# berkeley-hipie/HIPIE

Measured on AMD Instinct MI355X. Metric: images/sec @1024x1024 ViT-H bs=8 (single-image inference hot path: box, class and mask logits), higher is better.
Workload: dtype f16x3 (split-fp16 operands, fp32 accumulate: fp32-class); 1 GPU; BASELINE.json configs[2]: vit_huge, 1024x1024, batch 8 per GPU, 80 class prompts (L=194), detection; global_batch=8, parallelism=dp1, precision_policy=split, launch=eager

## Files before the change

### hipie_amd/csrc/vit_attn_split.hip

```cpp
#include <stdlib.h>

#include "common.h"
#include "mfma.h"
#include "wave.h"

#ifndef HIPIE_VS_TAIL
#define HIPIE_VS_TAIL 1
#endif
#ifndef HIPIE_VS_TAIL_MAXNB
#define HIPIE_VS_TAIL_MAXNB 3
#endif

namespace hipie {

constexpr float VS_LAZY = 6.f;

struct VSParams {
  const f16_t* qkv; f16_t* out; const f16_t* tab_h; const f16_t* tab_w;
  int B, H, N, kh, kw;
  long sb, st;
  long o_sb, o_st;
  int nqt, swz;
  int tr, kwm;
  long krs, kts;
};

template <int HD, int NB, int WAVES, int R, int KW, int BHC>
__global__ __launch_bounds__(WAVES * 64, (NB >= 3 ? 1 : 2)) void vit_attn_split_kernel(const VSParams p) {
  typedef f16_t T;
  constexpr int KT = 32 * NB;
  constexpr int KS = HD / 16;
  constexpr int DB = (HD + 31) / 32;
  constexpr int KSTR = HD + 8;
  constexpr int VSTR = (DB * 32 == 96 || DB * 32 == 32) ? DB * 32 : DB * 32 + 32;
  constexpr int CPR = HD / 8;
  constexpr int KCH = KSTR / 8, VCH = VSTR / 8;
  constexpr int KBLK = (KT * KCH + 63) / 64, VBLK = (KT * VCH + 63) / 64;
  constexpr int KPL = KBLK * 512, VPL = VBLK * 512;
  constexpr int BUF = 2 * KPL + 2 * VPL;
  constexpr int NBLK = 2 * KBLK + 2 * VBLK;
  constexpr int NDMA = (NBLK + WAVES - 1) / WAVES;
  constexpr int QW = WAVES * 32;
  constexpr int NT = WAVES * 64;
  constexpr bool TAIL = (HD % 32 == 16) && (HIPIE_VS_TAIL != 0) && NB <= HIPIE_VS_TAIL_MAXNB;
  constexpr int DBB = TAIL ? HD / 32 : DB;
  constexpr bool ONES = (DB * 32 > HD) && !TAIL;
  static_assert(R == 1 || (KW > 0 && R * KW <= KT), "R key rows of KW keys must fit the tile");
  static_assert(BHC == 0 || (R == 1 && BHC <= 31), "chunked bias_h: one key row per tile, at most 31 rows per chunk");
  static_assert(KSTR % 8 == 0 && VSTR % 8 == 0, "plane rows are whole 16-byte chunks");
  typedef Mfma32<T>::frag frag;
  typedef Mfma32<T>::half_frag hfrag;

  extern __shared__ __attribute__((aligned(1024))) char smem_raw[];
  T* smem = reinterpret_cast<T*>(smem_raw);
  constexpr size_t TILE_BYTES = ((size_t)2 * BUF * sizeof(T) > (size_t)WAVES * 4096) ? (size_t)2 * BUF * sizeof(T) : (size_t)WAVES * 4096;
  float* bh_all = reinterpret_cast<float*>(smem_raw + TILE_BYTES);

  const int tid = threadIdx.x, lane = tid & 63;
  const int wave = __builtin_amdgcn_readfirstlane(tid >> 6);
  const int li = lane & 31, hi = lane >> 5;
  const int kw = (R > 1) ? KW : p.kw, kh = p.kh;

  int bh, qt;
  {
    const int id = blockIdx.x;
    if (p.swz) { bh = (id & 7) + 8 * ((id >> 3) / p.nqt); qt = (id >> 3) % p.nqt; }
    else { bh = id / p.nqt; qt = id % p.nqt; }
  }
  const int b = bh / p.H, h = bh % p.H;
  const long C2 = 2L * p.H * HD;
  const T* Qg = p.qkv + b * p.sb + (long)h * (2 * HD);
  const T* Kg = Qg + C2;
  T* Og = p.out + b * p.o_sb + (long)h * (2 * HD);

  const int qi = qt * QW + wave * 32 + li;
  const int qc = min(qi, p.N - 1);
  const int qy = qc / kw, qx = qc - qy * kw;
  const long qm = p.tr ? (long)qx * p.kwm + qy : (long)qc;
  const int nkt = R * kw;

  frag qh[KS], ql[KS];
#pragma unroll
  for (int ks = 0; ks < KS; ++ks) {
    const T* s = Qg + qm * p.st + 16 * (2 * ks + hi);
    qh[ks] = *reinterpret_cast<const frag*>(s);
    ql[ks] = *reinterpret_cast<const frag*>(s + 8);
  }

  f32x16 bw[NB];
#pragma unroll
  for (int blk = 0; blk < NB; ++blk)
#pragma unroll
    for (int r = 0; r < 16; ++r) bw[blk][r] = -INFINITY;
  {
    float* stage = reinterpret_cast<float*>(smem_raw) + wave * (32 * 32);
    const int nbw = (2 * kw - 1 + 31) / 32, nbh = (2 * kh - 1 + 31) / 32;
    auto table_block = [&](const T* tab, const int rows, const int jb) -> f32x16 {
      f32x16 acc;
#pragma unroll
      for (int r = 0; r < 16; ++r) acc[r] = 0.f;
      const T* ap = tab + (long)min(32 * jb + li, rows - 1) * (2 * HD) + 16 * hi;
#pragma unroll
      for (int ks = 0; ks < KS; ++ks) {
        const frag th = *reinterpret_cast<const frag*>(ap + 32 * ks), tl = *reinterpret_cast<const frag*>(ap + 32 * ks + 8);
        acc = Mfma32<T>::mma(tl, qh[ks], acc);
        acc = Mfma32<T>::mma(th, ql[ks], acc);
        acc = Mfma32<T>::mma(th, qh[ks], acc);
      }
      return acc;
    };
    for (int jb = 0; jb < nbw; ++jb) {
      const f32x16 acc = table_block(p.tab_w, 2 * kw - 1, jb);
#pragma unroll
      for (int r = 0; r < 16; ++r) stage[crow(r, hi) * 32 + li] = acc[r];
      __syncthreads();
#pragma unroll
      for (int blk = 0; blk < NB; ++blk)
#pragma unroll
        for (int r = 0; r < 16; ++r) {
          const int slot = 32 * blk + crow(r, hi);
          const int kx = (R > 1) ? slot % kw : slot;
          const int j = qx + kw - 1 - kx - 32 * jb;
          if (slot < R * kw && j >= 0 && j < 32) bw[blk][r] = stage[j * 32 + li];
        }
      __syncthreads();
    }
    if (BHC == 0) {
      for (int jb = 0; jb < nbh; ++jb) {
        const f32x16 acc = table_block(p.tab_h, 2 * kh - 1, jb);
#pragma unroll
        for (int r = 0; r < 16; ++r) {
          const int ky = qy + kh - 1 - (32 * jb + crow(r, hi));
          if (ky >= 0 && ky < kh) bh_all[ky * QW + wave * 32 + li] = acc[r];
        }
      }
    }
    __syncthreads();
  }
  const int qy0 = __builtin_amdgcn_readfirstlane(qy);
  auto bias_h_chunk = [&](const int t0) {
    const int j0 = qy0 + kh - 1 - (t0 + BHC - 1);
    f32x16 acc;
#pragma unroll
    for (int r = 0; r < 16; ++r) acc[r] = 0.f;
    const T* ap = p.tab_h + (long)min(max(j0 + li, 0), 2 * kh - 2) * (2 * HD) + 16 * hi;
#pragma unroll
    for (int ks = 0; ks < KS; ++ks) {
      const frag th = *reinterpret_cast<const frag*>(ap + 32 * ks), tl = *reinterpret_cast<const frag*>(ap + 32 * ks + 8);
      acc = Mfma32<T>::mma(tl, qh[ks], acc);
      acc = Mfma32<T>::mma(th, ql[ks], acc);
      acc = Mfma32<T>::mma(th, qh[ks], acc);
    }
#pragma unroll
    for (int r = 0; r < 16; ++r) {
      const int ky = qy + kh - 1 - (j0 + crow(r, hi));
      if (ky >= t0 && ky < t0 + BHC && ky < kh) bh_all[(ky - t0) * QW + wave * 32 + li] = acc[r];
    }
  };

  const int nt = (kh + R - 1) / R;
  const bool ragged = (R > 1) && (nt * nkt > p.N);
  auto dma_voff = [&](const int r, const int maxrow) -> unsigned int {
    const int j = wave + WAVES * r;
    const int jj = min(j, NBLK - 1);
    const bool isk = jj < 2 * KBLK;
    const int pl = isk ? jj / KBLK : (jj - 2 * KBLK) / VBLK;
    const int c = 64 * (isk ? jj - pl * KBLK : jj - 2 * KBLK - pl * VBLK) + lane;
    const int nch = isk ? KCH : VCH;
    const int row = min(min(c / nch, KT - 1), maxrow);
    int col = c % nch;
    if (col >= CPR) col = 0;
    return (unsigned int)(((long)row * p.krs + (isk ? 0 : C2) + 16 * col + 8 * pl) * (long)sizeof(T));
  };
  unsigned int dvoff[NDMA];
  unsigned long long dmask[NDMA];
#pragma unroll
  for (int r = 0; r < NDMA; ++r) {
    dvoff[r] = dma_voff(r, nkt - 1);
    const int jj = min(wave + WAVES * r, NBLK - 1);
    const bool isk = jj < 2 * KBLK;
    const int pl = isk ? jj / KBLK : (jj - 2 * KBLK) / VBLK;
    const int c = 64 * (isk ? jj - pl * KBLK : jj - 2 * KBLK - pl * VBLK) + lane;
    dmask[r] = __builtin_amdgcn_ballot_w64(c % (isk ? KCH : VCH) < CPR);
  }
  const unsigned int lds0 = (unsigned int)reinterpret_cast<uintptr_t>((__attribute__((address_space(3))) char*)smem_raw);
  const char* kbase0 = reinterpret_cast<const char*>(Kg);
  const long tile_bytes = (R > 1 ? (long)nkt * p.st : p.kts) * (long)sizeof(T);
  auto dma_tile = [&](const int t, const int buf, const int r) {
    const int j = (WAVES * r + WAVES - 1 < NBLK) ? wave + WAVES * r : min(wave + WAVES * r, NBLK - 1);
    const bool last_ragged = ragged && (t == nt - 1);
    const unsigned int vo = last_ragged ? dma_voff(r, p.N - t * nkt - 1) : dvoff[r];
    const unsigned int ldst = __builtin_amdgcn_readfirstlane(lds0 + (unsigned int)(buf * BUF * (int)sizeof(T) + 1024 * j));
    dma16_masked(kbase0 + (long)t * tile_bytes, vo, ldst, dmask[r]);
  };

  {
    constexpr int PADC = VCH - CPR;
    for (int idx = tid; idx < 2 * 2 * KT * PADC; idx += NT) {
      const int pc = idx % PADC, row = (idx / PADC) % KT, pl = (idx / (PADC * KT)) & 1, buf = idx / (2 * PADC * KT);
      f16x8 z;
#pragma unroll
      for (int e = 0; e < 8; ++e) z[e] = (T)0.f;
      if (ONES && pl == 0 && pc == 0) z[0] = (T)1.f;
      *reinterpret_cast<f16x8*>(smem + buf * BUF + 2 * KPL + pl * VPL + row * VSTR + (CPR + pc) * 8) = z;
    }
  }

  f32x16 O[DBB];
  f32x4 OT[2];
  float m_run = -INFINITY, l_run = 0.f;
#pragma unroll
  for (int d = 0; d < DBB; ++d)
#pragma unroll
    for (int r = 0; r < 16; ++r) O[d][r] = 0.f;
#pragma unroll
  for (int r = 0; r < 4; ++r) { OT[0][r] = 0.f; OT[1][r] = 0.f; }

#pragma unroll
  for (int r = 0; r < NDMA; ++r) dma_tile(0, 0, r);
  __builtin_amdgcn_s_waitcnt(vmcnt(0));
  __syncthreads();

  const int l16 = lane & 15, g1 = (lane >> 4) & 1;
  const int vlane = (4 * hi + (l16 >> 2)) * VSTR + 16 * g1 + 4 * (l16 & 3);
  const int klane = li * KSTR + 8 * hi;

  for (int t = 0; t < nt; ++t) {
    const T* Kh = smem + (t & 1) * BUF;
    const T* Kl = Kh + KPL;
    const T* Vh = Kh + 2 * KPL;
    const T* Vl = Vh + VPL;
    const int tn = min(t + 1, nt - 1);
    if (BHC > 0 && t % (BHC > 0 ? BHC : 1) == 0) bias_h_chunk(t);
    float bh0 = bh_all[(BHC > 0 ? t % (BHC > 0 ? BHC : 1) : R * t) * QW + wave * 32 + li], bh1 = 0.f;
    if (R > 1) bh1 = (R * t + 1 < kh) ? bh_all[(R * t + 1) * QW + wave * 32 + li] : -INFINITY;

    f32x16 S[NB];
    {
      frag kfh[2][NB], kfl[2][NB];
#pragma unroll
      for (int blk = 0; blk < NB; ++blk) {
        kfh[0][blk] = *reinterpret_cast<const frag*>(Kh + klane + 32 * blk * KSTR);
        kfl[0][blk] = *reinterpret_cast<const frag*>(Kl + klane + 32 * blk * KSTR);
      }
#pragma unroll
      for (int ks = 0; ks < KS; ++ks) {
        if (ks + 1 < KS) {
#pragma unroll
          for (int blk = 0; blk < NB; ++blk) {
            kfh[(ks + 1) & 1][blk] = *reinterpret_cast<const frag*>(Kh + klane + 32 * blk * KSTR + 16 * (ks + 1));
            kfl[(ks + 1) & 1][blk] = *reinterpret_cast<const frag*>(Kl + klane + 32 * blk * KSTR + 16 * (ks + 1));
          }
        }
#pragma unroll
        for (int blk = 0; blk < NB; ++blk) {
          S[blk] = Mfma32<T>::mma(kfl[ks & 1][blk], qh[ks], (ks == 0) ? bw[blk] : S[blk]);
          S[blk] = Mfma32<T>::mma(kfh[ks & 1][blk], ql[ks], S[blk]);
          S[blk] = Mfma32<T>::mma(kfh[ks & 1][blk], qh[ks], S[blk]);
        }
        if (ks < NDMA) dma_tile(tn, (t + 1) & 1, ks);
      }
#pragma unroll
      for (int r = KS; r < NDMA; ++r) dma_tile(tn, (t + 1) & 1, r);
    }
    hfrag va[2][DBB], vb[2][DBB];
#pragma unroll
    for (int d = 0; d < DBB; ++d) {
      va[0][d] = Mfma32<T>::tr_read(Vh + vlane + 32 * d);
      vb[0][d] = Mfma32<T>::tr_read(Vh + vlane + 32 * d + 8 * VSTR);
    }

    if (R > 1) {
#pragma unroll
      for (int blk = 0; blk < NB; ++blk)
#pragma unroll
        for (int r = 0; r < 16; ++r) S[blk][r] += (32 * blk + crow(r, hi) < kw) ? bh0 : bh1;
    }
    float t0 = __builtin_fmaxf(S[0][0], S[0][1]);
#pragma unroll
    for (int blk = 1; blk < NB; ++blk) t0 = __builtin_fmaxf(t0, S[blk][0]);
    float mx = t0, mxb = t0, mxc = t0, mxd = t0;
#pragma unroll
    for (int blk = 0; blk < NB; ++blk)
#pragma unroll
      for (int r = 0; r < 16; r += 8) {
        mx = max3(mx, S[blk][r], S[blk][r + 1]);
        mxb = max3(mxb, S[blk][r + 2], S[blk][r + 3]);
        mxc = max3(mxc, S[blk][r + 4], S[blk][r + 5]);
        mxd = max3(mxd, S[blk][r + 6], S[blk][r + 7]);
      }
    mx = max3(mx, mxb, mxc);
    mx = max3(mx, mxd, mxd);
    mx = xhalf_max(mx);
    mx += (R > 1 ? 0.f : bh0);
    if (__builtin_amdgcn_ballot_w64(mx > m_run + VS_LAZY) != 0ull) {
      const float m_new = fmaxf(m_run, mx);
      const float alpha = __builtin_amdgcn_exp2f(m_run - m_new);
      m_run = m_new;
      if (!ONES) l_run *= alpha;
#pragma unroll
      for (int d = 0; d < DBB; ++d)
#pragma unroll
        for (int r = 0; r < 16; ++r) O[d][r] *= alpha;
      if (TAIL) {
        const float ax = __shfl(alpha, lane & 15), ay = __shfl(alpha, 16 + (lane & 15));
#pragma unroll
        for (int r = 0; r < 4; ++r) { OT[0][r] *= ax; OT[1][r] *= ay; }
      }
    }
    const float off = (R > 1 ? 0.f : bh0) - m_run;

    typedef unsigned int u32x4 __attribute__((ext_vector_type(4)));
    if constexpr (TAIL) {
      u32x4 p_h[2][2], p_l[2][2];
      auto make_p = [&](const int blk, const int st, u32x4& Hh, u32x4& Ll) {
        unsigned int hh[4], ll[4];
        float pv[8];
#pragma unroll
        for (int j = 0; j < 8; ++j) pv[j] = __builtin_amdgcn_exp2f(S[blk][8 * st + j] + off);
        exp_settle(pv);
#pragma unroll
        for (int j = 0; j < 4; ++j) {
          l_run += pv[2 * j] + pv[2 * j + 1];
          hl_split2(pv[2 * j], pv[2 * j + 1], hh[j], ll[j]);
        }
        settle(hh, ll);
#pragma unroll
        for (int j = 0; j < 4; ++j) { Hh[j] = hh[j]; Ll[j] = ll[j]; }
      };
      const int tg = lane >> 4, tj = lane & 15;
      const int tlane = ((tg & 1) * 16 + (tg >> 1) * 4 + (tj >> 2)) * VSTR + 32 * DBB + 4 * (tj & 3);
      hfrag ta_h[2], ta_l[2];
      make_p(0, 0, p_h[0][0], p_l[0][0]);
#pragma unroll
      for (int u = 0; u < 4 * NB; ++u) {
        const int step = u >> 1, pl = u & 1, blk = step >> 1, st = step & 1, bp = blk & 1;
        frag vf[DBB];
#pragma unroll
        for (int d = 0; d < DBB; ++d)
#pragma unroll
          for (int j = 0; j < 4; ++j) { vf[d][j] = va[u & 1][d][j]; vf[d][4 + j] = vb[u & 1][d][j]; }
        if (u + 1 < 4 * NB) {
          const int nstep = (u + 1) >> 1, npl = (u + 1) & 1;
          const T* vbp = (npl ? Vl : Vh) + (16 * nstep) * VSTR + vlane;
#pragma unroll
          for (int d = 0; d < DBB; ++d) {
            va[(u + 1) & 1][d] = Mfma32<T>::tr_read(vbp + 32 * d);
            vb[(u + 1) & 1][d] = Mfma32<T>::tr_read(vbp + 32 * d + 8 * VSTR);
          }
          if (npl == 0) make_p(nstep >> 1, nstep & 1, p_h[(nstep >> 1) & 1][nstep & 1], p_l[(nstep >> 1) & 1][nstep & 1]);
        }
        if (st == 1 && pl == 0) {
          ta_h[0] = Mfma32<T>::tr_read(Vh + (32 * blk) * VSTR + tlane);
          ta_h[1] = Mfma32<T>::tr_read(Vh + (32 * blk + 8) * VSTR + tlane);
          ta_l[0] = Mfma32<T>::tr_read(Vl + (32 * blk) * VSTR + tlane);
          ta_l[1] = Mfma32<T>::tr_read(Vl + (32 * blk + 8) * VSTR + tlane);
        }
        const frag pf = __builtin_bit_cast(frag, p_h[bp][st]);
#pragma unroll
        for (int d = 0; d < DBB; ++d) O[d] = Mfma32<T>::mma(vf[d], pf, O[d]);
        if (pl == 0) {
          const frag pfl = __builtin_bit_cast(frag, p_l[bp][st]);
#pragma unroll
          for (int d = 0; d < DBB; ++d) O[d] = Mfma32<T>::mma(vf[d], pfl, O[d]);
        }
        if (st == 1 && pl == 1) {
          typedef unsigned int u32x2 __attribute__((ext_vector_type(2)));
          u32x4 xh, yh, xl, yl;
#pragma unroll
          for (int j = 0; j < 4; ++j) {
            const u32x2 sh = __builtin_amdgcn_permlane16_swap(p_h[bp][0][j], p_h[bp][1][j], false, false);
            const u32x2 sl = __builtin_amdgcn_permlane16_swap(p_l[bp][0][j], p_l[bp][1][j], false, false);
            xh[j] = sh[0]; yh[j] = sh[1]; xl[j] = sl[0]; yl[j] = sl[1];
          }
          frag ah, al;
#pragma unroll
          for (int j = 0; j < 4; ++j) { ah[j] = ta_h[0][j]; ah[4 + j] = ta_h[1][j]; al[j] = ta_l[0][j]; al[4 + j] = ta_l[1][j]; }
          const frag fxh = __builtin_bit_cast(frag, xh), fyh = __builtin_bit_cast(frag, yh);
          OT[0] = __builtin_amdgcn_mfma_f32_16x16x32_f16(ah, fxh, OT[0], 0, 0, 0);
          OT[1] = __builtin_amdgcn_mfma_f32_16x16x32_f16(ah, fyh, OT[1], 0, 0, 0);
          OT[0] = __builtin_amdgcn_mfma_f32_16x16x32_f16(ah, __builtin_bit_cast(frag, xl), OT[0], 0, 0, 0);
          OT[1] = __builtin_amdgcn_mfma_f32_16x16x32_f16(ah, __builtin_bit_cast(frag, yl), OT[1], 0, 0, 0);
          OT[0] = __builtin_amdgcn_mfma_f32_16x16x32_f16(al, fxh, OT[0], 0, 0, 0);
          OT[1] = __builtin_amdgcn_mfma_f32_16x16x32_f16(al, fyh, OT[1], 0, 0, 0);
        }
      }
    } else {
    frag pf, pfl;
    {
      unsigned int hh[4], ll[4];
      float pv[8];
#pragma unroll
      for (int j = 0; j < 8; ++j) pv[j] = __builtin_amdgcn_exp2f(S[0][j] + off);
      exp_settle(pv);
#pragma unroll
      for (int j = 0; j < 4; ++j) {
        if (!ONES) l_run += pv[2 * j] + pv[2 * j + 1];
        hl_split2(pv[2 * j], pv[2 * j + 1], hh[j], ll[j]);
      }
      settle(hh, ll);
      pf = __builtin_bit_cast(frag, (u32x4){hh[0], hh[1], hh[2], hh[3]});
      pfl = __builtin_bit_cast(frag, (u32x4){ll[0], ll[1], ll[2], ll[3]});
    }
#pragma unroll
    for (int u = 0; u < 4 * NB; ++u) {
      const int step = u >> 1, pl = u & 1;
      frag vf[DB];
#pragma unroll
      for (int d = 0; d < DB; ++d)
#pragma unroll
        for (int j = 0; j < 4; ++j) { vf[d][j] = va[u & 1][d][j]; vf[d][4 + j] = vb[u & 1][d][j]; }
      frag pn = pf, pnl = pfl;
      if (u + 1 < 4 * NB) {
        const int nstep = (u + 1) >> 1, npl = (u + 1) & 1;
        const T* vbp = (npl ? Vl : Vh) + (16 * nstep) * VSTR + vlane;
#pragma unroll
        for (int d = 0; d < DB; ++d) {
          va[(u + 1) & 1][d] = Mfma32<T>::tr_read(vbp + 32 * d);
          vb[(u + 1) & 1][d] = Mfma32<T>::tr_read(vbp + 32 * d + 8 * VSTR);
        }
        if (npl == 0) {
          const int nb_ = nstep >> 1, ns_ = nstep & 1;
          unsigned int hh[4], ll[4];
          float pv[8];
#pragma unroll
          for (int j = 0; j < 8; ++j) pv[j] = __builtin_amdgcn_exp2f(S[nb_][8 * ns_ + j] + off);
          exp_settle(pv);
#pragma unroll
          for (int j = 0; j < 4; ++j) {
            if (!ONES) l_run += pv[2 * j] + pv[2 * j + 1];
            hl_split2(pv[2 * j], pv[2 * j + 1], hh[j], ll[j]);
          }
          settle(hh, ll);
          pn = __builtin_bit_cast(frag, (u32x4){hh[0], hh[1], hh[2], hh[3]});
          pnl = __builtin_bit_cast(frag, (u32x4){ll[0], ll[1], ll[2], ll[3]});
        }
      }
#pragma unroll
      for (int d = 0; d < DB; ++d) O[d] = Mfma32<T>::mma(vf[d], pf, O[d]);
      if (pl == 0) {
#pragma unroll
        for (int d = 0; d < DB; ++d) O[d] = Mfma32<T>::mma(vf[d], pfl, O[d]);
      }
      pf = pn;
      pfl = pnl;
      (void)step;
    }

    }

    __builtin_amdgcn_s_waitcnt(vmcnt(0));
    __syncthreads();
  }

  {
    static_assert(!ONES || (HD % 32 == 16), "the ones column is read back from O^T row 16 of the last block");
    const float l_tot = ONES ? __shfl(O[DBB - 1][8], li) : l_run + __shfl_xor(l_run, 32);
    const float inv = 1.f / l_tot;
    if (qi < p.N) {
      T* orow = Og + qm * p.o_st;
#pragma unroll
      for (int d = 0; d < DBB; ++d)
#pragma unroll
        for (int rr = 0; rr < 4; ++rr) {
          const int d0 = 32 * d + 8 * rr + 4 * hi;
          if (d0 < HD) {
            f16x4 oh, ol;
#pragma unroll
            for (int e = 0; e < 4; ++e) {
              T hh, ll;
              hl_split(O[d][4 * rr + e] * inv, hh, ll);
              oh[e] = hh;
              ol[e] = ll;
            }
            T* dst = orow + 16 * (d0 >> 3) + 4 * hi;
            *reinterpret_cast<f16x4*>(dst) = oh;
            *reinterpret_cast<f16x4*>(dst + 8) = ol;
          }
        }
    }
    if (TAIL) {
      const int d0 = 32 * DBB + 4 * (lane >> 4);
#pragma unroll
      for (int h2 = 0; h2 < 2; ++h2) {
        const int ql = 16 * h2 + (lane & 15);
        const float iv = __shfl(inv, ql);
        const int qi2 = qt * QW + wave * 32 + ql;
        const int qc2 = min(qi2, p.N - 1);
        const int qy2 = qc2 / kw, qx2 = qc2 - qy2 * kw;
        const long qm2 = p.tr ? (long)qx2 * p.kwm + qy2 : (long)qc2;
        if (qi2 < p.N) {
          f16x4 oh, ol;
#pragma unroll
          for (int e = 0; e < 4; ++e) {
            T hh, ll;
            hl_split(OT[h2][e] * iv, hh, ll);
            oh[e] = hh;
            ol[e] = ll;
          }
          T* dst = Og + qm2 * p.o_st + 16 * (d0 >> 3) + (d0 & 4);
          *reinterpret_cast<f16x4*>(dst) = oh;
          *reinterpret_cast<f16x4*>(dst + 8) = ol;
        }
      }
    }
  }
}

template <int HD, int NB, int WAVES, int R, int KW, int BHC = 0>
static int launch_vs(VSParams& p, hipStream_t st) {
  constexpr int KT = 32 * NB, DB = (HD + 31) / 32;
  constexpr int KSTR = HD + 8, VSTR = (DB * 32 == 96 || DB * 32 == 32) ? DB * 32 : DB * 32 + 32;
  constexpr int KBLK = (KT * (KSTR / 8) + 63) / 64, VBLK = (KT * (VSTR / 8) + 63) / 64;
  size_t lds = (size_t)2 * (2 * KBLK + 2 * VBLK) * 1024;
  const size_t stage = (size_t)WAVES * 32 * 32 * sizeof(float);
  if (lds < stage) lds = stage;
  lds += (size_t)(BHC > 0 ? BHC : p.kh) * WAVES * 32 * sizeof(float);
  if (lds > 160 * 1024) return set_err(HIPIE_EINVAL, "vit_attn(split): %zu bytes of LDS needed (grid %dx%d) > 160 KiB", lds, p.kh, p.kw);
  p.nqt = (p.N + WAVES * 32 - 1) / (WAVES * 32);
  p.swz = ((p.B * p.H) % 8 == 0) ? 1 : 0;
  const unsigned grid = (unsigned)(p.nqt * p.B * p.H);
  auto kern = vit_attn_split_kernel<HD, NB, WAVES, R, KW, BHC>;
  static LdsLimit limit;
  limit.raise((const void*)kern, lds, 64 * 1024);
  hipLaunchKernelGGL(kern, dim3(grid), dim3(WAVES * 64), lds, st, p);
  return check_launch("vit_attn(split)");
}

template <int HD>
static int dispatch_vs(VSParams& p, hipStream_t st) {
  if (p.kw == 14 && p.kh <= 96) return launch_vs<HD, 1, 7, 2, 14>(p, st);
  if (p.kw <= 32) return launch_vs<HD, 1, 4, 1, 0>(p, st);
  if (p.kw <= 64 && p.kh <= 64) return launch_vs<HD, 2, 8, 1, 0>(p, st);
  if (p.kw <= 64) return launch_vs<HD, 2, 4, 1, 0>(p, st);
  if (p.kw <= 96) return launch_vs<HD, 3, 8, 1, 0, 16>(p, st);
  return set_err(HIPIE_EINVAL, "vit_attn(split): token grids wider than 96 in BOTH directions are not supported (got %dx%d)", p.kh, p.kw);
}

}

extern "C" int hipie_vit_attn_split(const void* qkv, const void* tab_h, const void* tab_w, void* out, int B, int gh, int gw,
                                    int heads, int hd, void* stream) {
  using namespace hipie;
  HIPIE_REQUIRE(qkv && out && tab_h && tab_w, "vit_attn_split: null pointer");
  HIPIE_REQUIRE((((uintptr_t)qkv | (uintptr_t)out | (uintptr_t)tab_h | (uintptr_t)tab_w) & 15) == 0, "vit_attn_split: pointers must be 16-byte aligned");
  HIPIE_REQUIRE(B > 0 && gh > 0 && gw > 0 && heads > 0, "vit_attn_split: bad shape B=%d grid %dx%d heads=%d", B, gh, gw, heads);
  HIPIE_REQUIRE(gh <= 160, "vit_attn_split: more than 160 key rows (%d) are not supported", gh);
  const long N = (long)gh * gw, C = (long)heads * hd;
  HIPIE_REQUIRE(N * 6 * C * 2 < (1L << 31), "vit_attn_split: an image's qkv block must stay below 2 GiB");
  VSParams p{};
  p.qkv = (const f16_t*)qkv; p.out = (f16_t*)out; p.tab_h = (const f16_t*)tab_h; p.tab_w = (const f16_t*)tab_w;
  p.B = B; p.H = heads; p.N = (int)N; p.kh = gh; p.kw = gw;
  p.sb = N * 6 * C; p.st = 6 * C; p.o_sb = N * 2 * C; p.o_st = 2 * C;
  p.tr = 0; p.kwm = gw; p.krs = p.st; p.kts = (long)gw * p.st;
  {
    static int force_tr = -1;
    if (force_tr < 0) { const char* e = study_env("HIPIE_VA_TRANSPOSE"); force_tr = e ? atoi(e) : 0; }
    if ((gw > 96 && gh <= 96) || (force_tr == 1 && gw != 14)) {
      p.tr = 1; p.kh = gw; p.kw = gh; p.tab_h = (const f16_t*)tab_w; p.tab_w = (const f16_t*)tab_h;
      p.krs = (long)gw * p.st; p.kts = p.st;
    }
  }
  hipStream_t st = (hipStream_t)stream;
  if (hd == 80) return dispatch_vs<80>(p, st);
  if (hd == 64) return dispatch_vs<64>(p, st);
  return set_err(HIPIE_EINVAL, "vit_attn_split: head_dim 64 / 80 only (got %d)", hd);
}
```

Before: 43.38 images/sec.

## Compute split attention PV product entirely with 16x16 MFMA blocks for head dim 80

```diff
diff --git a/hipie_amd/csrc/vit_attn_split.hip b/hipie_amd/csrc/vit_attn_split.hip
--- a/hipie_amd/csrc/vit_attn_split.hip
+++ b/hipie_amd/csrc/vit_attn_split.hip
@@ -25,7 +25,7 @@
   long krs, kts;
 };
 
-template <int HD, int NB, int WAVES, int R, int KW, int BHC>
+template <int HD, int NB, int WAVES, int R, int KW, int BHC, bool PV16>
 __global__ __launch_bounds__(WAVES * 64, (NB >= 3 ? 1 : 2)) void vit_attn_split_kernel(const VSParams p) {
   typedef f16_t T;
   constexpr int KT = 32 * NB;
@@ -42,9 +42,13 @@
   constexpr int NDMA = (NBLK + WAVES - 1) / WAVES;
   constexpr int QW = WAVES * 32;
   constexpr int NT = WAVES * 64;
-  constexpr bool TAIL = (HD % 32 == 16) && (HIPIE_VS_TAIL != 0) && NB <= HIPIE_VS_TAIL_MAXNB;
-  constexpr int DBB = TAIL ? HD / 32 : DB;
-  constexpr bool ONES = (DB * 32 > HD) && !TAIL;
+  constexpr bool TAIL = !PV16 && (HD % 32 == 16) && (HIPIE_VS_TAIL != 0) && NB <= HIPIE_VS_TAIL_MAXNB;
+  constexpr int DBB = PV16 ? 0 : TAIL ? HD / 32 : DB;
+  constexpr int DBA = DBB > 0 ? DBB : 1;
+  constexpr int NE = PV16 ? HD / 16 : 1;
+  constexpr int TB0 = PV16 ? 0 : 32 * DBB;
+  constexpr bool ONES = (DB * 32 > HD) && !TAIL && !PV16;
+  static_assert(!PV16 || HD % 16 == 0, "PV16: the head dim is a whole number of 16-row blocks");
   static_assert(R == 1 || (KW > 0 && R * KW <= KT), "R key rows of KW keys must fit the tile");
   static_assert(BHC == 0 || (R == 1 && BHC <= 31), "chunked bias_h: one key row per tile, at most 31 rows per chunk");
   static_assert(KSTR % 8 == 0 && VSTR % 8 == 0, "plane rows are whole 16-byte chunks");
@@ -194,7 +198,7 @@
     dma16_masked(kbase0 + (long)t * tile_bytes, vo, ldst, dmask[r]);
   };
 
-  {
+  if constexpr (!PV16) {
     constexpr int PADC = VCH - CPR;
     for (int idx = tid; idx < 2 * 2 * KT * PADC; idx += NT) {
       const int pc = idx % PADC, row = (idx / PADC) % KT, pl = (idx / (PADC * KT)) & 1, buf = idx / (2 * PADC * KT);
@@ -206,15 +210,17 @@
     }
   }
 
-  f32x16 O[DBB];
-  f32x4 OT[2];
+  f32x16 O[DBA];
+  f32x4 OT[NE][2];
   float m_run = -INFINITY, l_run = 0.f;
 #pragma unroll
   for (int d = 0; d < DBB; ++d)
 #pragma unroll
     for (int r = 0; r < 16; ++r) O[d][r] = 0.f;
 #pragma unroll
-  for (int r = 0; r < 4; ++r) { OT[0][r] = 0.f; OT[1][r] = 0.f; }
+  for (int e = 0; e < NE; ++e)
+#pragma unroll
+    for (int r = 0; r < 4; ++r) { OT[e][0][r] = 0.f; OT[e][1][r] = 0.f; }
 
 #pragma unroll
   for (int r = 0; r < NDMA; ++r) dma_tile(0, 0, r);
@@ -224,6 +230,15 @@
   const int l16 = lane & 15, g1 = (lane >> 4) & 1;
   const int vlane = (4 * hi + (l16 >> 2)) * VSTR + 16 * g1 + 4 * (l16 & 3);
   const int klane = li * KSTR + 8 * hi;
+  typedef hfrag hfrag4[4];
+  auto pv16_reads = [lane](const T* Vh_, const T* Vl_, const int blk, const int e, hfrag4& a) {
+    const int tg = lane >> 4, tj = lane & 15;
+    const int tlane = ((tg & 1) * 16 + (tg >> 1) * 4 + (tj >> 2)) * VSTR + TB0 + 4 * (tj & 3);
+    a[0] = Mfma32<T>::tr_read(Vh_ + (32 * blk) * VSTR + tlane + 16 * e);
+    a[1] = Mfma32<T>::tr_read(Vh_ + (32 * blk + 8) * VSTR + tlane + 16 * e);
+    a[2] = Mfma32<T>::tr_read(Vl_ + (32 * blk) * VSTR + tlane + 16 * e);
+    a[3] = Mfma32<T>::tr_read(Vl_ + (32 * blk + 8) * VSTR + tlane + 16 * e);
+  };
 
   for (int t = 0; t < nt; ++t) {
     const T* Kh = smem + (t & 1) * BUF;
@@ -263,12 +278,14 @@
 #pragma unroll
       for (int r = KS; r < NDMA; ++r) dma_tile(tn, (t + 1) & 1, r);
     }
-    hfrag va[2][DBB], vb[2][DBB];
+    hfrag va[2][DBA], vb[2][DBA];
 #pragma unroll
     for (int d = 0; d < DBB; ++d) {
       va[0][d] = Mfma32<T>::tr_read(Vh + vlane + 32 * d);
       vb[0][d] = Mfma32<T>::tr_read(Vh + vlane + 32 * d + 8 * VSTR);
     }
+    hfrag4 ta16[2];
+    if constexpr (PV16) pv16_reads(Vh, Vl, 0, 0, ta16[0]);
 
     if (R > 1) {
 #pragma unroll
@@ -302,16 +319,18 @@
       for (int d = 0; d < DBB; ++d)
 #pragma unroll
         for (int r = 0; r < 16; ++r) O[d][r] *= alpha;
-      if (TAIL) {
+      if (TAIL || PV16) {
         const float ax = __shfl(alpha, lane & 15), ay = __shfl(alpha, 16 + (lane & 15));
 #pragma unroll
-        for (int r = 0; r < 4; ++r) { OT[0][r] *= ax; OT[1][r] *= ay; }
+        for (int e = 0; e < NE; ++e)
+#pragma unroll
+          for (int r = 0; r < 4; ++r) { OT[e][0][r] *= ax; OT[e][1][r] *= ay; }
       }
     }
     const float off = (R > 1 ? 0.f : bh0) - m_run;
 
     typedef unsigned int u32x4 __attribute__((ext_vector_type(4)));
-    if constexpr (TAIL) {
+    if constexpr (TAIL || PV16) {
       u32x4 p_h[2][2], p_l[2][2];
       auto make_p = [&](const int blk, const int st, u32x4& Hh, u32x4& Ll) {
         unsigned int hh[4], ll[4];
@@ -328,9 +347,46 @@
 #pragma unroll
         for (int j = 0; j < 4; ++j) { Hh[j] = hh[j]; Ll[j] = ll[j]; }
       };
-      const int tg = lane >> 4, tj = lane & 15;
-      const int tlane = ((tg & 1) * 16 + (tg >> 1) * 4 + (tj >> 2)) * VSTR + 32 * DBB + 4 * (tj & 3);
-      hfrag ta_h[2], ta_l[2];
+      typedef unsigned int u32x2 __attribute__((ext_vector_type(2)));
+      auto redeal = [&p_h, &p_l](const int bp, u32x4& xh, u32x4& yh, u32x4& xl, u32x4& yl) {
+#pragma unroll
+        for (int j = 0; j < 4; ++j) {
+          const u32x2 sh = __builtin_amdgcn_permlane16_swap(p_h[bp][0][j], p_h[bp][1][j], false, false);
+          const u32x2 sl = __builtin_amdgcn_permlane16_swap(p_l[bp][0][j], p_l[bp][1][j], false, false);
+          xh[j] = sh[0]; yh[j] = sh[1]; xl[j] = sl[0]; yl[j] = sl[1];
+        }
+      };
+      auto pv16_block = [](const hfrag4& a, const u32x4& xh, const u32x4& yh, const u32x4& xl, const u32x4& yl, f32x4 (&acc)[2]) {
+        frag ah, al;
+#pragma unroll
+        for (int j = 0; j < 4; ++j) { ah[j] = a[0][j]; ah[4 + j] = a[1][j]; al[j] = a[2][j]; al[4 + j] = a[3][j]; }
+        const frag fxh = __builtin_bit_cast(frag, xh), fyh = __builtin_bit_cast(frag, yh);
+        acc[0] = Mfma16<T>::mma(ah, fxh, acc[0]);
+        acc[1] = Mfma16<T>::mma(ah, fyh, acc[1]);
+        acc[0] = Mfma16<T>::mma(ah, __builtin_bit_cast(frag, xl), acc[0]);
+        acc[1] = Mfma16<T>::mma(ah, __builtin_bit_cast(frag, yl), acc[1]);
+        acc[0] = Mfma16<T>::mma(al, fxh, acc[0]);
+        acc[1] = Mfma16<T>::mma(al, fyh, acc[1]);
+      };
+      if constexpr (PV16) {
+        make_p(0, 0, p_h[0][0], p_l[0][0]);
+        make_p(0, 1, p_h[0][1], p_l[0][1]);
+#pragma unroll
+        for (int blk = 0; blk < NB; ++blk) {
+          const int bp = blk & 1;
+          u32x4 xh, yh, xl, yl;
+          redeal(bp, xh, yh, xl, yl);
+#pragma unroll
+          for (int e = 0; e < NE; ++e) {
+            const int i = blk * NE + e;
+            if (i + 1 < NB * NE) pv16_reads(Vh, Vl, (i + 1) / NE, (i + 1) % NE, ta16[(i + 1) & 1]);
+            if (blk + 1 < NB && e == 0) make_p(blk + 1, 0, p_h[bp ^ 1][0], p_l[bp ^ 1][0]);
+            if (blk + 1 < NB && e == NE / 2) make_p(blk + 1, 1, p_h[bp ^ 1][1], p_l[bp ^ 1][1]);
+            pv16_block(ta16[i & 1], xh, yh, xl, yl, OT[e]);
+          }
+        }
+      } else {
+      hfrag4 ta;
       make_p(0, 0, p_h[0][0], p_l[0][0]);
 #pragma unroll
       for (int u = 0; u < 4 * NB; ++u) {
@@ -350,12 +406,7 @@
           }
           if (npl == 0) make_p(nstep >> 1, nstep & 1, p_h[(nstep >> 1) & 1][nstep & 1], p_l[(nstep >> 1) & 1][nstep & 1]);
         }
-        if (st == 1 && pl == 0) {
-          ta_h[0] = Mfma32<T>::tr_read(Vh + (32 * blk) * VSTR + tlane);
-          ta_h[1] = Mfma32<T>::tr_read(Vh + (32 * blk + 8) * VSTR + tlane);
-          ta_l[0] = Mfma32<T>::tr_read(Vl + (32 * blk) * VSTR + tlane);
-          ta_l[1] = Mfma32<T>::tr_read(Vl + (32 * blk + 8) * VSTR + tlane);
-        }
+        if (st == 1 && pl == 0) pv16_reads(Vh, Vl, blk, 0, ta);
         const frag pf = __builtin_bit_cast(frag, p_h[bp][st]);
 #pragma unroll
         for (int d = 0; d < DBB; ++d) O[d] = Mfma32<T>::mma(vf[d], pf, O[d]);
@@ -365,25 +416,11 @@
           for (int d = 0; d < DBB; ++d) O[d] = Mfma32<T>::mma(vf[d], pfl, O[d]);
         }
         if (st == 1 && pl == 1) {
-          typedef unsigned int u32x2 __attribute__((ext_vector_type(2)));
           u32x4 xh, yh, xl, yl;
-#pragma unroll
-          for (int j = 0; j < 4; ++j) {
-            const u32x2 sh = __builtin_amdgcn_permlane16_swap(p_h[bp][0][j], p_h[bp][1][j], false, false);
-            const u32x2 sl = __builtin_amdgcn_permlane16_swap(p_l[bp][0][j], p_l[bp][1][j], false, false);
-            xh[j] = sh[0]; yh[j] = sh[1]; xl[j] = sl[0]; yl[j] = sl[1];
-          }
-          frag ah, al;
-#pragma unroll
-          for (int j = 0; j < 4; ++j) { ah[j] = ta_h[0][j]; ah[4 + j] = ta_h[1][j]; al[j] = ta_l[0][j]; al[4 + j] = ta_l[1][j]; }
-          const frag fxh = __builtin_bit_cast(frag, xh), fyh = __builtin_bit_cast(frag, yh);
-          OT[0] = __builtin_amdgcn_mfma_f32_16x16x32_f16(ah, fxh, OT[0], 0, 0, 0);
-          OT[1] = __builtin_amdgcn_mfma_f32_16x16x32_f16(ah, fyh, OT[1], 0, 0, 0);
-          OT[0] = __builtin_amdgcn_mfma_f32_16x16x32_f16(ah, __builtin_bit_cast(frag, xl), OT[0], 0, 0, 0);
-          OT[1] = __builtin_amdgcn_mfma_f32_16x16x32_f16(ah, __builtin_bit_cast(frag, yl), OT[1], 0, 0, 0);
-          OT[0] = __builtin_amdgcn_mfma_f32_16x16x32_f16(al, fxh, OT[0], 0, 0, 0);
-          OT[1] = __builtin_amdgcn_mfma_f32_16x16x32_f16(al, fyh, OT[1], 0, 0, 0);
-        }
+          redeal(bp, xh, yh, xl, yl);
+          pv16_block(ta, xh, yh, xl, yl, OT[0]);
+        }
+      }
       }
     } else {
     frag pf, pfl;
@@ -455,7 +492,7 @@
 
   {
     static_assert(!ONES || (HD % 32 == 16), "the ones column is read back from O^T row 16 of the last block");
-    const float l_tot = ONES ? __shfl(O[DBB - 1][8], li) : l_run + __shfl_xor(l_run, 32);
+    const float l_tot = ONES ? __shfl(O[DBA - 1][8], li) : l_run + __shfl_xor(l_run, 32);
     const float inv = 1.f / l_tot;
     if (qi < p.N) {
       T* orow = Og + qm * p.o_st;
@@ -479,35 +516,40 @@
           }
         }
     }
-    if (TAIL) {
-      const int d0 = 32 * DBB + 4 * (lane >> 4);
+    if (TAIL || PV16) {
+      int kwe = kw;
+      if constexpr (PV16 && NB >= 3) asm volatile("" : "+s"(kwe));
 #pragma unroll
       for (int h2 = 0; h2 < 2; ++h2) {
         const int ql = 16 * h2 + (lane & 15);
         const float iv = __shfl(inv, ql);
         const int qi2 = qt * QW + wave * 32 + ql;
         const int qc2 = min(qi2, p.N - 1);
-        const int qy2 = qc2 / kw, qx2 = qc2 - qy2 * kw;
+        const int qy2 = qc2 / kwe, qx2 = qc2 - qy2 * kwe;
         const long qm2 = p.tr ? (long)qx2 * p.kwm + qy2 : (long)qc2;
         if (qi2 < p.N) {
-          f16x4 oh, ol;
-#pragma unroll
-          for (int e = 0; e < 4; ++e) {
-            T hh, ll;
-            hl_split(OT[h2][e] * iv, hh, ll);
-            oh[e] = hh;
-            ol[e] = ll;
+#pragma unroll
+          for (int e = 0; e < NE; ++e) {
+            const int d0 = TB0 + 16 * e + 4 * (lane >> 4);
+            f16x4 oh, ol;
+#pragma unroll
+            for (int r = 0; r < 4; ++r) {
+              T hh, ll;
+              hl_split(OT[e][h2][r] * iv, hh, ll);
+              oh[r] = hh;
+              ol[r] = ll;
+            }
+            T* dst = Og + qm2 * p.o_st + 16 * (d0 >> 3) + (d0 & 4);
+            *reinterpret_cast<f16x4*>(dst) = oh;
+            *reinterpret_cast<f16x4*>(dst + 8) = ol;
           }
-          T* dst = Og + qm2 * p.o_st + 16 * (d0 >> 3) + (d0 & 4);
-          *reinterpret_cast<f16x4*>(dst) = oh;
-          *reinterpret_cast<f16x4*>(dst + 8) = ol;
         }
       }
     }
   }
 }
 
-template <int HD, int NB, int WAVES, int R, int KW, int BHC = 0>
+template <int HD, int NB, int WAVES, int R, int KW, int BHC, bool PV16>
 static int launch_vs(VSParams& p, hipStream_t st) {
   constexpr int KT = 32 * NB, DB = (HD + 31) / 32;
   constexpr int KSTR = HD + 8, VSTR = (DB * 32 == 96 || DB * 32 == 32) ? DB * 32 : DB * 32 + 32;
@@ -520,20 +562,31 @@
   p.nqt = (p.N + WAVES * 32 - 1) / (WAVES * 32);
   p.swz = ((p.B * p.H) % 8 == 0) ? 1 : 0;
   const unsigned grid = (unsigned)(p.nqt * p.B * p.H);
-  auto kern = vit_attn_split_kernel<HD, NB, WAVES, R, KW, BHC>;
+  auto kern = vit_attn_split_kernel<HD, NB, WAVES, R, KW, BHC, PV16>;
   static LdsLimit limit;
   limit.raise((const void*)kern, lds, 64 * 1024);
   hipLaunchKernelGGL(kern, dim3(grid), dim3(WAVES * 64), lds, st, p);
   return check_launch("vit_attn(split)");
 }
 
+static inline bool vs_pv16(const bool shipped) {
+  const char* e = study_env("HIPIE_VS_PV");
+  return e ? atoi(e) == 16 : shipped;
+}
+
+template <int HD, int NB, int WAVES, int R, int KW, int BHC = 0>
+static int launch_vs_pv(VSParams& p, hipStream_t st, const bool shipped16) {
+  return vs_pv16(shipped16) ? launch_vs<HD, NB, WAVES, R, KW, BHC, true>(p, st) : launch_vs<HD, NB, WAVES, R, KW, BHC, false>(p, st);
+}
+
 template <int HD>
 static int dispatch_vs(VSParams& p, hipStream_t st) {
-  if (p.kw == 14 && p.kh <= 96) return launch_vs<HD, 1, 7, 2, 14>(p, st);
-  if (p.kw <= 32) return launch_vs<HD, 1, 4, 1, 0>(p, st);
-  if (p.kw <= 64 && p.kh <= 64) return launch_vs<HD, 2, 8, 1, 0>(p, st);
-  if (p.kw <= 64) return launch_vs<HD, 2, 4, 1, 0>(p, st);
-  if (p.kw <= 96) return launch_vs<HD, 3, 8, 1, 0, 16>(p, st);
+  constexpr bool W16 = HD == 80, G16 = HD == 80, X16 = HD == 80;
+  if (p.kw == 14 && p.kh <= 96) return launch_vs_pv<HD, 1, 7, 2, 14>(p, st, W16);
+  if (p.kw <= 32) return launch_vs_pv<HD, 1, 4, 1, 0>(p, st, false);
+  if (p.kw <= 64 && p.kh <= 64) return launch_vs_pv<HD, 2, 8, 1, 0>(p, st, G16);
+  if (p.kw <= 64) return launch_vs_pv<HD, 2, 4, 1, 0>(p, st, false);
+  if (p.kw <= 96) return launch_vs_pv<HD, 3, 8, 1, 0, 16>(p, st, X16);
   return set_err(HIPIE_EINVAL, "vit_attn(split): token grids wider than 96 in BOTH directions are not supported (got %dx%d)", p.kh, p.kw);
 }
 
```

Result: no change. 43.16 images/sec (-0.5%).
